# ZhiHuangHn/vtkCloudPoint

Hardware: AMD Instinct MI355X
Metric: Mpoints/s DBSCAN+label @10M pts (higher is better)
Workload: dtype f64; 1 GPU; C4: 10000000-pt cloud (half uniform background, 200 Gaussian blobs), one monolithic DBImproved.dbscan, metric L1_2D, eps 0.1, minPts 10; mode=single, points_total=10000000, points_per_gpu=10000000, clusters=27380, resident_in_hbm=True

## Files before the change

vtkcloudpoint_amd/csrc/dbscan.hip:

```cpp
#include <string.h>

#include <cmath>
#include <cstdlib>
#include <cstring>
#include <limits>
#include <vector>

#include "bounds.hpp"
#include "dbscan_engine.hpp"
#include "grid_common.hpp"

using namespace vcpg;

namespace {

#ifndef VCP_UNR2
#define VCP_UNR2 4
#endif
#ifndef VCP_UNR3
#define VCP_UNR3 2
#endif
#ifndef VCP_UNRW
#define VCP_UNRW 4
#endif

}

struct SlabState {
// ... 91 lines not shown
  for (int r = 0; r < NR; r++) {
    const int y = cc[1] + (r % 3) - 1;
    const int z = GD == 3 ? cc[2] + (r / 3) - 1 : 0;
    const bool ok = y >= 0 && y < g.D[1] && (GD != 3 || (z >= 0 && z < g.D[2]));
    const uint32_t base = ok ? cell_id<GD>(g, 0, y, z) : 0u;
    rs[r] = re[r] = 0u;
    if (ok) ct_range(ct, base + x0, base + x1 + 1, rs[r], re[r]);
  }
}

constexpr unsigned XCHUNK = 8;
constexpr unsigned LCHUNK = 1;
__device__ __forceinline__ int64_t xcd_block(unsigned nblocks) {
  const unsigned b = blockIdx.x;
  const unsigned per = nblocks / (8u * XCHUNK);
  if (b >= per * 8u * XCHUNK) return b;
  const unsigned x = b & 7u, i = b >> 3;
  return (int64_t)((i / per) * 8u + x) * per + (i % per);
}

struct WorkList {
  uint32_t* list;
  const uint32_t* scan;
  uint32_t perblk;
  uint32_t nblk;
};

__device__ __forceinline__ uint32_t wl_fetch(const WorkList& w) {
  const uint32_t total = w.scan[w.nblk] - w.scan[0];
  const uint32_t x = blockIdx.x & 7u, i = blockIdx.x >> 3;
  const uint32_t c = (i / w.perblk) * 8u + x;
  const uint32_t lo = (uint32_t)(((uint64_t)total * c) / (8u * LCHUNK));
  const uint32_t hi = (uint32_t)(((uint64_t)total * (c + 1u)) / (8u * LCHUNK));
  const uint32_t t = lo + (i % w.perblk) * TPB + threadIdx.x;
  if (t >= hi) return NONE;
  return w.list[t];
}

__device__ __forceinline__ void wl_count(bool isE, bool isB, uint32_t blk, uint32_t* __restrict__ cntE,
                                         uint32_t* __restrict__ cntB) {
  __shared__ unsigned wc[2][TPB / 64];
  const unsigned long long mE = __ballot(isE), mB = __ballot(isB);
  if ((threadIdx.x & 63) == 0) {
    wc[0][threadIdx.x >> 6] = (unsigned)__popcll(mE);
    wc[1][threadIdx.x >> 6] = (unsigned)__popcll(mB);
  }
  __syncthreads();
  if (threadIdx.x == 0) {
    unsigned a = 0, b = 0;
    for (int k = 0; k < TPB / 64; k++) {
      a += wc[0][k];
      b += wc[1][k];
    }
    cntE[blk] = a;
    cntB[blk] = b;
  }
}

__global__ __launch_bounds__(TPB) void k_wl_fill(const uint8_t* __restrict__ flags, CellTab ct, const uint32_t* __restrict__ scanE,
// ... 470 lines not shown
  for_rows<GD>(cc, g, ct, [&](uint32_t s, uint32_t e) {
    if (s >= me) return true;
    if (e > me) e = me;
    for (uint32_t j0 = s; j0 < e; j0 += UNR) {
      float rr[UNR][3];
      bool cand[UNR];
#pragma unroll
      for (int u = 0; u < UNR; u++) {
        const uint32_t jj = min(j0 + u, e - 1);
        cand[u] = (j0 + u < e) && (flags[jj] & F_EXPAND);
        if (GROUPED) cand[u] = cand[u] && sgroup[jj] == myg;
        load_pt32<GD>(sorted32, jj, rr[u]);
      }
#pragma unroll
      for (int u = 0; u < UNR; u++)
        if (first == me && cand[u] && within_scr<GD, METRIC>(qf, rr[u], sc, xs, me, j0 + u, thr)) first = j0 + u;
      if (first != me) return false;
    }
    return true;
  });
  if (first != me) parent[me] = first;
}

__global__ __launch_bounds__(TPB) void k_union_init_list(const uint8_t* __restrict__ flags, uint32_t* __restrict__ parent,
                                                        NbrOut no, WorkList wlE) {
  const uint32_t p = wl_fetch(wlE);
  if (p == NONE) return;
  const int nrec = flags[p] >> 4;
  const uint32_t* li = nbr_list(no, p);
  for (int k = 0; k < nrec; k++) {
    const uint32_t j = li[k];
    if (j < p && (flags[j] & F_EXPAND)) {
      parent[p] = j;
      return;
    }
  }
}

template <int JOIN>
__global__ __launch_bounds__(TPB) void k_flatten0(uint32_t* __restrict__ parent, WorkList wlE,
                                                 const uint8_t* __restrict__ flags, NbrOut no) {
  const uint32_t p = wl_fetch(wlE);
  if (p == NONE) return;
  uint32_t r = (uint32_t)p, x = ld_parent_cached(parent, r);
  if (x == r || JOIN == 2) {
    if (!JOIN) return;
    uint32_t rp = JOIN == 2 ? uf_root(parent, p) : p;
    const int nrec = flags[p] >> 4;
    const uint32_t* li = nbr_list(no, p);
    uint32_t s0 = NONE, s1 = NONE, s2 = NONE;
    for (int k = 0; k < nrec; k++) {
      const uint32_t j = li[k];
      if (!(flags[j] & F_EXPAND)) continue;
      const uint32_t y = ld_parent_cached(parent, j);
      if (y == rp || y == s0 || y == s1 || y == s2) continue;
      const uint32_t ry = uf_root(parent, y);
      const uint32_t rm = uf_root(parent, rp);
      s2 = s1;
      s1 = s0;
      s0 = rp;
      rp = (ry != rm) ? uf_link(parent, rm, ry) : rm;
      if (y != rp) s1 = y;
    }
    return;
  }
  while (x != r) {
    r = x;
    x = ld_parent_cached(parent, r);
  }
  __hip_atomic_store(&parent[p], r, __ATOMIC_RELAXED, __HIP_MEMORY_SCOPE_WAVEFRONT);
}

constexpr uint32_t CHUNK_MIXED = 0xFFFFFFFEu;
constexpr int DENSE_PER_CELL = 16;
__global__ __launch_bounds__(TPB) void k_chunkroot(const uint32_t* __restrict__ parent, CellTab ct,
                                                  uint32_t* __restrict__ chunkroot) {
  const uint32_t nin = *ct.nin;
  const int64_t p = (int64_t)blockIdx.x * TPB + threadIdx.x;
  const uint32_t x = p < nin ? parent[p] : NONE;
  const unsigned long long have = __ballot(x != NONE);
  uint32_t out = NONE;
  if (have) {
    const uint32_t r = (uint32_t)__shfl((int)x, __ffsll((long long)have) - 1, 64);
    out = __ballot(x != NONE && x != r) ? CHUNK_MIXED : r;
  }
  if ((threadIdx.x & 63) == 0) chunkroot[p >> 6] = out;
}

#define VCP_JOIN(x)                                                \
  do {                                                             \
    const uint32_t rx__ = uf_root(parent, (x));                    \
    const uint32_t rm__ = uf_root(parent, rp);                     \
    rp = (rx__ != rm__) ? uf_link(parent, rm__, rx__) : rm__;      \
// ... 74 lines not shown
          if (x2 != rp) {
            const uint32_t rx = uf_root(parent, x2);
            const uint32_t rm = uf_root(parent, rp);
            rp = (rx != rm) ? uf_link(parent, rm, rx) : rm;
          }
          if (x != rp && j != rp) __hip_atomic_store(&parent[j], rp, __ATOMIC_RELAXED, __HIP_MEMORY_SCOPE_WAVEFRONT);
        } else if (q0 == NONE) {
          q0 = x;
        } else if (q1 == NONE) {
          q1 = x;
        } else {
          VCP_FLUSH();
          q0 = x;
        }
      }
    }
  }
  VCP_FLUSH();
  if (rp != me) __hip_atomic_store(&parent[me], rp, __ATOMIC_RELAXED, __HIP_MEMORY_SCOPE_AGENT);
}
#undef VCP_FLUSH
#undef VCP_JOIN

template <bool FILTER>
__global__ __launch_bounds__(TPB) void k_flatten(uint32_t* __restrict__ parent, const uint32_t* __restrict__ sord,
                                                uint32_t* __restrict__ minord, WorkList wlE) {
  const uint32_t p = wl_fetch(wlE);
  uint32_t r = NONE, v = NONE;
  if (p != NONE) {
    r = (uint32_t)p;
    uint32_t x = parent[r];
    while (x != r) {
      r = x;
      x = parent[r];
    }
    parent[p] = r;
    v = sord[p];
  }
  unsigned long long todo = __ballot(r != NONE);
  const int lane = threadIdx.x & 63;
  while (todo) {
    int leader = __ffsll((long long)todo) - 1;
    uint32_t lr = __shfl(r, leader, 64);
    bool mine = (r == lr);
    uint32_t m = mine ? v : NONE;
#pragma unroll
    for (int d = 32; d > 0; d >>= 1) m = min(m, (uint32_t)__shfl_xor((int)m, d, 64));
    if (lane == leader &&
        (!FILTER || m < __hip_atomic_load(&minord[lr], __ATOMIC_RELAXED, __HIP_MEMORY_SCOPE_AGENT)))
      atomicMin(&minord[lr], m);
    todo &= ~__ballot(mine);
  }
}

__device__ __forceinline__ uint32_t seed_rank(const uint32_t* __restrict__ bits, const uint32_t* __restrict__ pref,
                                              uint32_t m) {
  const uint32_t w = m >> 5;
  return pref[w] + (uint32_t)__popc(bits[w] & ((1u << (m & 31u)) - 1u));
}
__global__ __launch_bounds__(TPB) void k_seed_popc(const uint32_t* __restrict__ bits, uint32_t nw, uint32_t* __restrict__ cnt) {
  uint32_t w = blockIdx.x * TPB + threadIdx.x;
  if (w < nw) cnt[w] = (uint32_t)__popc(bits[w]);
}

__global__ __launch_bounds__(TPB) void k_seedflag(const uint32_t* __restrict__ parent, const uint32_t* __restrict__ minord,
                                                 uint32_t* __restrict__ seedflag, WorkList wlE) {
  const uint32_t p = wl_fetch(wlE);
  if (p == NONE) return;
  if (parent[p] == p) {
    const uint32_t m = minord[p];
    atomicOr(&seedflag[m >> 5], 1u << (m & 31u));
  }
}

__global__ __launch_bounds__(TPB) void k_rootk(const uint32_t* __restrict__ parent, const uint32_t* __restrict__ minord,
                                              const uint32_t* __restrict__ seedbits, const uint32_t* __restrict__ seedpref,
                                              uint32_t* __restrict__ rootk, uint32_t* __restrict__ clseed, WorkList wlE) {
  const uint32_t p = wl_fetch(wlE);
  if (p == NONE) return;
  if (parent[p] == p) {
    uint32_t k = seed_rank(seedbits, seedpref, minord[p]);
    rootk[p] = k;
    clseed[k] = minord[p];
  }
}

__device__ __forceinline__ void twice_add(unsigned twice, unsigned long long* __restrict__ counters) {
  __shared__ unsigned tw[TPB / 64];
  const unsigned long long m2 = __ballot(twice);
  if ((threadIdx.x & 63) == 0) tw[threadIdx.x >> 6] = (unsigned)__popcll(m2);
  __syncthreads();
  if (threadIdx.x == 0) {
    unsigned t = 0;
    for (int k = 0; k < TPB / 64; k++) t += tw[k];
    if (t) atomicAdd(&counters[CNT_TWICE + (blockIdx.x & (CNT_SPREAD - 1))], (unsigned long long)t);
  }
}

template <int GD, int METRIC, bool GROUPED>
__global__ __launch_bounds__(TPB) void k_border(ExactSrc xs, GridP g, double thr,
                                               CellTab ct,
                                               const int32_t* __restrict__ sgroup, const uint8_t* __restrict__ flags,
                                               const uint32_t* __restrict__ parent, const uint32_t* __restrict__ sord,
                                               const uint32_t* __restrict__ rootk, const uint32_t* __restrict__ clseed,
                                               uint32_t* __restrict__ labk, unsigned long long* __restrict__ counters,
                                               uint32_t* __restrict__ group_twice, WorkList wlB, uint32_t own_lo,
                                               uint32_t own_span, const float* __restrict__ sorted32, Screen sc) {
  const uint32_t p = wl_fetch(wlB);
  unsigned twice = 0;
  if (p != NONE) {
    const uint8_t fl = flags[p];
    uint32_t out = 0;
    {
// ... 15 lines not shown
            if (j >= e || x == NONE || (x >= mnk && x < mx)) continue;
            if (GROUPED && sgroup[j] != myg) continue;
            float rr[3];
            load_pt32<GD>(sorted32, j, rr);
            if (within_scr<GD, METRIC>(qf, rr, sc, xs, p, j, thr)) {
              mx = max(mx, x + 1u);
              mnk = min(mnk, x);
            }
          }
        }
        return true;
      });
      out = mx;
      if (mx != 0 && !(fl & F_CLASSED) && sord[p] - own_lo < own_span && sord[p] < clseed[mnk]) {
        twice = 1;
        if (GROUPED) atomicAdd(&group_twice[myg], 1u);
      }
    }
    labk[p] = (out << 2) | ((fl & F_CORE) ? 1u : 0u) | ((fl & F_CLASSED) ? 2u : 0u);
  }
  if (!GROUPED) twice_add(twice, counters);
}

template <bool GROUPED>
__global__ __launch_bounds__(TPB) void k_border_list(const int32_t* __restrict__ sgroup, const uint8_t* __restrict__ flags,
                                                    const uint32_t* __restrict__ sord, const uint32_t* __restrict__ rootk,
                                                    const uint32_t* __restrict__ clseed, uint32_t* __restrict__ labk,
                                                    unsigned long long* __restrict__ counters,
                                                    uint32_t* __restrict__ group_twice, NbrOut no, WorkList wlB) {
  const uint32_t p = wl_fetch(wlB);
  unsigned twice = 0;
  if (p != NONE) {
    const uint8_t fl = flags[p];
    const int nrec = fl >> 4;
    uint32_t mx = 0, mnk = NONE;
    const uint32_t* li = nbr_list(no, p);
    for (int k = 0; k < nrec; k++) {
      const uint32_t x = rootk[li[k]];
      if (x == NONE) continue;
      mx = max(mx, x + 1u);
      mnk = min(mnk, x);
    }
    if (mx != 0 && sord[p] < clseed[mnk]) twice = 1;
    labk[p] = (mx << 2) | ((fl & F_CORE) ? 1u : 0u) | ((fl & F_CLASSED) ? 2u : 0u);
  }
  if (GROUPED) {
    const int32_t g = twice ? sgroup[p] : -1;
    unsigned long long todo = __ballot(twice != 0);
    const int lane = threadIdx.x & 63;
    while (todo) {
      const int leader = __ffsll((long long)todo) - 1;
      const int32_t gl = __shfl(g, leader, 64);
      const unsigned long long same = __ballot(twice && g == gl);
      if (lane == leader) atomicAdd(&group_twice[gl], (uint32_t)__popcll(same));
      todo &= ~same;
    }
  } else {
    twice_add(twice, counters);
  }
}

__global__ __launch_bounds__(TPB) void k_labk_rest(const uint8_t* __restrict__ flags, const uint32_t* __restrict__ parent,
                                                  uint32_t* rootk, uint32_t* __restrict__ labk,
                                                  CellTab ct) {
  const uint32_t nin = *ct.nin;
  int64_t p = (int64_t)blockIdx.x * TPB + threadIdx.x;
  if (p >= nin) return;
  const uint8_t fl = flags[p];
  uint32_t k = NONE;
  if (fl & F_EXPAND) {
    const uint32_t r = parent[p];
    k = rootk[r];
    if (r != (uint32_t)p) rootk[p] = k;
  } else {
    rootk[p] = NONE;
  }
  if (fl & F_BCAND) return;
  const uint32_t out = (fl & F_EXPAND) ? k + 1u : 0u;
  labk[p] = (out << 2) | ((fl & F_CORE) ? 1u : 0u) | ((fl & F_CLASSED) ? 2u : 0u);
}

// ... 223 lines not shown
  if (metric == VCP_L1_2D) {
    err = 2.0 * alpha * (1.0 + u) + 2.0 * u * (1.0 + u) * thr;
  } else {
    err = 2.0 * alpha * std::sqrt((double)gd * thr) * (1.0 + u) + (double)gd * alpha * alpha + 6.0 * u * (1.0 + u) * thr;
    lo_ok = std::sqrt(thr) > 4.0 * alpha * std::sqrt((double)gd);
  }
  err = err * 1.0625 + 1e-14 * thr + 1e-300;
  const double lo = thr - err, hi = thr + err;
  if (std::isfinite(hi)) {
    float h = (float)hi;
    if ((double)h < hi) h = std::nextafterf(h, INFINITY);
    sc.hi = h;
  }
  if (lo_ok && lo >= 0.0 && std::isfinite(lo)) {
    float l = (float)lo;
    if ((double)l > lo) l = std::nextafterf(l, -INFINITY);
    sc.lo = l;
  } else if (lo_ok && std::isinf(thr) && thr > 0) {
    sc.lo = 3.4028234663852886e38f;
  }
  return sc;
}

unsigned list_perblk(int64_t n) {
  const int64_t band = (n + 8 * LCHUNK - 1) / (8 * LCHUNK) + 1;
  return vcp_blocks(band, TPB);
}

struct Switches {
  int64_t cells_per_point;
  bool screen_off, lists_off, core_global;
  int core_cap, join_all;
};
const Switches& switches() {
  static const Switches sw = [] {
    Switches s;
    const char* e = getenv("VCP_CELL_BUDGET");
    const long v = e ? atol(e) : 32;
    s.cells_per_point = (int64_t)(v < 1 ? 1 : v > 4096 ? 4096 : v);
    s.screen_off = getenv("VCP_NO_SCREEN") != nullptr;
    s.lists_off = getenv("VCP_NO_LISTS") != nullptr;
    s.core_global = getenv("VCP_CORE_GLOBAL") != nullptr;
    s.core_cap = getenv("VCP_CORE_CAP") ? atoi(getenv("VCP_CORE_CAP")) : -1;
    s.join_all = getenv("VCP_JOIN_ALL") ? atoi(getenv("VCP_JOIN_ALL")) : -1;
    return s;
  }();
  return sw;
}

struct EnginePinned {
  double bounds[8];
  uint32_t unclassed;
  uint32_t n_comp;
  unsigned long long counters[CNT_WORDS];
};
static_assert(sizeof(EnginePinned) <= 1024, "the engine's region of vcp_ctx::pinned");
EnginePinned* engine_pinned(vcp_ctx* ctx) { return reinterpret_cast<EnginePinned*>(ctx->pinned); }

struct Call {
  const double* d_coords;
  int64_t n;
  int stride, metric;
  double eps;
  int min_pts;
  int32_t cf_in;
  const uint8_t* d_in_classed;
  int32_t* d_labels;
  uint8_t *d_is_core, *d_is_classed;
  int32_t* cf_out;
  int64_t* dist_evals;
// ... 29 lines not shown
}
BoundsSrc bounds_src(const Call& c) { return BoundsSrc{c.d_coords, c.n, c.gd, c.stride, c.d_group, c.glo, c.ghi}; }

struct MiscView {
  double* d_part;
  double* d_bounds;
  unsigned long long* counters;
  uint32_t* d_total;
};
struct Workspace : MiscView {
  uint4* ctwords;
  uint32_t* ctdense;
  uint32_t* ctcount;
  CellTab ct;
  uint32_t *cellof, *pos, *sord, *parent, *minord, *rootk, *clseed, *labk;
  float* sorted32;
  uint8_t* flags;
  int32_t* sgroup;
  uint32_t nw;
  uint32_t* seedflag;
  uint32_t* seedpref;
  uint32_t *blkE, *blkB;
  WorkList wlE, wlB;
  unsigned nbl;
};

int ws_reserve_misc(vcp_ctx* ctx, int64_t n) {
  return vcp_ensure(ctx, ctx->b_misc, (size_t)(vcp_bounds_parts(n) * 8 + 96) * sizeof(double));
}
MiscView misc_carve(vcp_ctx* ctx, int64_t n) {
  MiscView m;
  m.d_part = ctx->b_misc.as<double>();
  m.d_bounds = m.d_part + (size_t)vcp_bounds_parts(n) * 8;
  m.counters = reinterpret_cast<unsigned long long*>(m.d_bounds + 8);
  m.d_total = reinterpret_cast<uint32_t*>(m.counters + CNT_SEED_TOTAL);
  return m;
}
static_assert((8 + CNT_WORDS) <= 96, "b_misc: bounds and counters behind the partials");

int ws_reserve(vcp_ctx* ctx, int64_t n, unsigned nb, int gd, bool grouped, uint32_t ncells) {
  const size_t ctw = vcp_ct_words(ncells), ctd = vcp_ct_dense_cap(n, ncells);
  VCP_TRY(vcp_ensure(ctx, ctx->b_ctw, ctw * 16 + 64));
  VCP_TRY(vcp_ensure(ctx, ctx->b_ctd, ctd * 128));
  VCP_TRY(vcp_ensure(ctx, ctx->b_cellof, (size_t)n * 4));
  VCP_TRY(vcp_ensure(ctx, ctx->b_pos, (size_t)n * 4));
  VCP_TRY(vcp_ensure(ctx, ctx->b_sorted32, (size_t)n * (gd == 2 ? 2 : 4) * 4));
  VCP_TRY(vcp_ensure(ctx, ctx->b_sidx, (size_t)n * 4));
// ... 17 lines not shown
  w.ctcount = reinterpret_cast<uint32_t*>(ctx->b_ctw.as<char>() + vcp_ct_words(ncells) * 16);
  w.ct = CellTab{w.ctwords, w.ctdense, w.ctcount + 1};
  w.cellof = ctx->b_cellof.as<uint32_t>();
  w.pos = ctx->b_pos.as<uint32_t>();
  w.sorted32 = ctx->b_sorted32.as<float>();
  w.sord = ctx->b_sidx.as<uint32_t>();
  w.flags = ctx->b_flags.as<uint8_t>();
  w.parent = ctx->b_parent.as<uint32_t>();
  w.minord = ctx->b_minord.as<uint32_t>();
  w.nw = (uint32_t)(n / 32 + 2);
  w.seedflag = ctx->b_seedflag.as<uint32_t>();
  w.seedpref = w.seedflag + ((w.nw + 3) & ~3u);
  w.rootk = ctx->b_rootcl.as<uint32_t>();
  w.clseed = ctx->b_clseed.as<uint32_t>();
  w.labk = ctx->b_labk.as<uint32_t>();
  w.sgroup = grouped ? ctx->b_sgroup.as<int32_t>() : nullptr;
  w.blkE = ctx->b_wl.as<uint32_t>();
  w.blkB = w.blkE + (nb + 2);
  w.wlE.list = w.blkB + (nb + 2);
  w.wlB.list = w.wlE.list + n;
  w.wlE.scan = w.blkE;
  w.wlB.scan = w.blkB;
  w.wlE.nblk = w.wlB.nblk = nb;
  w.wlE.perblk = w.wlB.perblk = list_perblk(n);
  w.nbl = 8u * LCHUNK * w.wlE.perblk;
  return w;
}

struct Totals {
  uint32_t K;
  unsigned long long unclassed;
  unsigned long long twice;
  unsigned long long slot0;
  unsigned long long group_evals;
};
int read_totals(vcp_ctx* ctx, const MiscView& ws, Totals& t) {
  unsigned long long* hc = engine_pinned(ctx)->counters;
  VCP_HIP(ctx, hipMemcpyAsync(hc, ws.counters, CNT_WORDS * sizeof(unsigned long long), hipMemcpyDeviceToHost, ctx->stream));
  VCP_TRY(vcp_phase_finish(ctx));
  VCP_HIP(ctx, hipStreamSynchronize(ctx->stream));
  t.K = *reinterpret_cast<uint32_t*>(hc + CNT_SEED_TOTAL);
  t.slot0 = hc[CNT_LONELY];
  t.group_evals = hc[CNT_GROUP_EVALS];
  t.unclassed = t.twice = 0;
  for (int k = 0; k < CNT_SPREAD; k++) {
    t.unclassed += hc[CNT_UNCLASSED + k];
    t.twice += hc[CNT_TWICE + k];
  }
// ... 178 lines not shown
  }
  const size_t lds_nb = (size_t)no.NB * TPB * 4;
  bool tiled = false;
  if constexpr (GD == 2) {
    if (!GROUPED || !sw.core_global) {
      VCP_LAUNCH(ctx, (k_core_lds<GD, METRIC, GROUPED>), dim3(nb), dim3(TPB), 0, st, c.xs, c.g, c.thr, c.min_pts, ws.ct,
                      ws.sgroup, ws.flags, ws.parent, ws.minord, ws.blkE, ws.blkB, no, ws.sorted32, c.sc, c.flags_set);
      tiled = true;
    }
  }
  if (!tiled)
    VCP_LAUNCH(ctx, (k_core<GD, METRIC, GROUPED>), dim3(nb), dim3(TPB), 2 * lds_nb, st, c.xs, c.g, c.thr, c.min_pts, ws.ct,
                    ws.sgroup, ws.flags, ws.parent, ws.minord, ws.blkE, ws.blkB, no, ws.sorted32, c.sc, c.flags_set);
  VCP_TRY(vcp_exclusive_scan_u32(ctx, ws.blkE, ws.blkE, 2 * ((int64_t)nb + 2), nullptr));
  VCP_LAUNCH(ctx, k_wl_fill, dim3(nb), dim3(TPB), 0, st, ws.flags, ws.ct, ws.blkE, ws.blkB, ws.wlE.list, ws.wlB.list,
                  ws.seedflag, ws.nw, ws.counters, c.d_group_twice, (uint32_t)(GROUPED ? c.G : 0));
  return VCP_OK;
}

template <int GD, int METRIC, bool GROUPED>
int stage_union(vcp_ctx* ctx, const Call& c, const Workspace& ws, const Switches& sw) {
  hipStream_t st = ctx->stream;
  const int64_t n = c.n;
  const unsigned nb = c.nb, nbl = ws.nbl;
  const GridP& g = c.g;
  const NbrOut& no = c.no;
  vcp_phase(ctx, "union");
  const bool pre = GD == 2 || no.NB > 0;
  if (no.NB > 0) {
    VCP_LAUNCH(ctx, k_union_init_list, dim3(nbl), dim3(TPB), 0, st, ws.flags, ws.parent, no, ws.wlE);
    const bool all = sw.join_all >= 0 ? sw.join_all != 0 : (uint64_t)n >= (uint64_t)g.ncells;
    if (all) VCP_LAUNCH(ctx, k_flatten0<2>, dim3(nbl), dim3(TPB), 0, st, ws.parent, ws.wlE, ws.flags, no);
    else VCP_LAUNCH(ctx, k_flatten0<1>, dim3(nbl), dim3(TPB), 0, st, ws.parent, ws.wlE, ws.flags, no);
    VCP_LAUNCH(ctx, k_flatten0<0>, dim3(nbl), dim3(TPB), 0, st, ws.parent, ws.wlE, ws.flags, no);
  } else if (GD == 2) {
    VCP_LAUNCH(ctx, (k_union_init<GD, METRIC, GROUPED>), dim3(nbl), dim3(TPB), 0, st, c.xs, g, c.thr, ws.ct, ws.sgroup,
                    ws.flags, ws.parent, ws.wlE, ws.sorted32, c.sc);
    VCP_LAUNCH(ctx, k_flatten0<0>, dim3(nbl), dim3(TPB), 0, st, ws.parent, ws.wlE, ws.flags, no);
  }
  const bool dense = pre && (uint64_t)n > (uint64_t)DENSE_PER_CELL * g.ncells;
  if (dense) {
    VCP_TRY(vcp_ensure(ctx, ctx->b_aux0, ((size_t)nb * (TPB / 64) + 2) * 4));
    uint32_t* chunkroot = ctx->b_aux0.as<uint32_t>();
    VCP_LAUNCH(ctx, k_chunkroot, dim3(nb), dim3(TPB), 0, st, ws.parent, ws.ct, chunkroot);
    VCP_LAUNCH(ctx, (k_union<GD, METRIC, GROUPED, true, true>), dim3(nbl), dim3(TPB), 0, st, c.xs, g, c.thr, ws.ct,
                    ws.sgroup, ws.parent, ws.wlE, ws.sorted32, c.sc, chunkroot);
  } else if (pre)
    VCP_LAUNCH(ctx, (k_union<GD, METRIC, GROUPED, true>), dim3(nbl), dim3(TPB), 0, st, c.xs, g, c.thr, ws.ct, ws.sgroup,
                    ws.parent, ws.wlE, ws.sorted32, c.sc);
  else
    VCP_LAUNCH(ctx, (k_union<GD, METRIC, GROUPED, false>), dim3(nbl), dim3(TPB), 0, st, c.xs, g, c.thr, ws.ct, ws.sgroup,
                    ws.parent, ws.wlE, ws.sorted32, c.sc);
  return VCP_OK;
}

int stage_slab_handoff(vcp_ctx* ctx, const Call& c, const Workspace& ws) {
  hipStream_t st = ctx->stream;
  const unsigned nb = c.nb;
  vcp_phase(ctx, "slab_components");
  VCP_LAUNCH(ctx, k_slab_count, dim3(nb), dim3(TPB), 0, st, ws.parent, ws.flags, ws.ct, ws.blkE);
  VCP_TRY(vcp_exclusive_scan_u32(ctx, ws.blkE, ws.blkE, (int64_t)nb + 1, nullptr));
// ... 1 lines not shown
  VCP_LAUNCH(ctx, k_slab_out, dim3(nb), dim3(TPB), 0, st, c.n, ws.pos, ws.flags, ws.parent, ws.minord, c.ext->d_slab_rep,
                  c.d_is_core);
  uint32_t* hn = &engine_pinned(ctx)->n_comp;
  VCP_HIP(ctx, hipMemcpyAsync(hn, ws.blkE + nb, 4, hipMemcpyDeviceToHost, st));
  VCP_TRY(vcp_phase_finish(ctx));
  VCP_HIP(ctx, hipStreamSynchronize(st));
  if (!ctx->slab) ctx->slab = new SlabState();
  SlabState& ss = *ctx->slab;
  ss.valid = true;
  ss.gd = c.gd;
  ss.metric = c.metric;
  ss.n = c.n;
  ss.n_comp = hn[0];
  ss.g = c.g;
  ss.thr = c.thr;
  ss.sc = c.sc;
  ss.xs = c.xs;
  ss.nb = nb;
  if (c.cf_out) *c.cf_out = (int32_t)hn[0];
  return VCP_OK;
}

template <bool GROUPED>
int stage_flatten_number(vcp_ctx* ctx, const Call& c, const Workspace& ws) {
  hipStream_t st = ctx->stream;
  const unsigned nbl = ws.nbl;
  vcp_phase(ctx, "flatten_number");
  if ((uint64_t)c.n >= (uint64_t)c.g.ncells)
    VCP_LAUNCH(ctx, k_flatten<true>, dim3(nbl), dim3(TPB), 0, st, ws.parent, ws.sord, ws.minord, ws.wlE);
  else
    VCP_LAUNCH(ctx, k_flatten<false>, dim3(nbl), dim3(TPB), 0, st, ws.parent, ws.sord, ws.minord, ws.wlE);
  if (!GROUPED && c.slab) return stage_slab_handoff(ctx, c, ws);
  VCP_LAUNCH(ctx, k_seedflag, dim3(nbl), dim3(TPB), 0, st, ws.parent, ws.minord, ws.seedflag, ws.wlE);
  VCP_LAUNCH(ctx, k_seed_popc, dim3(vcp_blocks(ws.nw, TPB)), dim3(TPB), 0, st, ws.seedflag, ws.nw, ws.seedpref);
  VCP_TRY(vcp_exclusive_scan_u32(ctx, ws.seedpref, ws.seedpref, ws.nw, ws.d_total));
  VCP_LAUNCH(ctx, k_rootk, dim3(nbl), dim3(TPB), 0, st, ws.parent, ws.minord, ws.seedflag, ws.seedpref, ws.rootk, ws.clseed,
                  ws.wlE);
  return VCP_OK;
}

template <int GD, int METRIC, bool GROUPED>
int stage_border(vcp_ctx* ctx, const Call& c, const Workspace& ws) {
  hipStream_t st = ctx->stream;
  vcp_phase(ctx, "border");
  VCP_LAUNCH(ctx, k_labk_rest, dim3(c.nb), dim3(TPB), 0, st, ws.flags, ws.parent, ws.rootk, ws.labk, ws.ct);
  if (c.no.NB > 0)
    VCP_LAUNCH(ctx, k_border_list<GROUPED>, dim3(ws.nbl), dim3(TPB), 0, st, ws.sgroup, ws.flags, ws.sord, ws.rootk,
                    ws.clseed, ws.labk, ws.counters, c.d_group_twice, c.no, ws.wlB);
  else
    VCP_LAUNCH(ctx, (k_border<GD, METRIC, GROUPED>), dim3(ws.nbl), dim3(TPB), 0, st, c.xs, c.g, c.thr, ws.ct, ws.sgroup,
                    ws.flags, ws.parent, ws.sord, ws.rootk, ws.clseed, ws.labk, ws.counters, c.d_group_twice, ws.wlB, 0u,
                    NONE, ws.sorted32, c.sc);
  return VCP_OK;
}

template <int GD, bool GROUPED>
int stage_output(vcp_ctx* ctx, const Call& c, const Workspace& ws) {
  hipStream_t st = ctx->stream;
  const int64_t n = c.n;
  const unsigned nb = c.nb;
  const DbscanExt* ext = c.ext;
  if (c.part_out) {
    GridOutputArgs oa;
    oa.n = n;
    oa.sord = ws.sord;
    oa.labk = ws.labk;
    oa.have_in_classed = c.d_in_classed != nullptr;
    oa.cf_in = c.cf_in;
    oa.labels = c.d_labels;
    oa.is_core = c.d_is_core;
    oa.is_classed = c.d_is_classed;
    oa.counters = ws.counters;
    VCP_TRY(vcp_grid_output_partition(ctx, oa));
// ... 15 lines not shown
  }
  return VCP_OK;
}

template <int GD, int METRIC, bool GROUPED>
int run_dbscan(vcp_ctx* ctx, Call& c) {
  const Switches& sw = switches();
  VCP_TRY(stage_bounds(ctx, c));
  c.thr = (METRIC == VCP_L1_2D) ? c.eps : l2_threshold(c.eps);
  if (!GROUPED && c.all_finite && !c.slab && box_measure<GD, METRIC>(c.h) <= c.thr) return run_all_pairs(ctx, c);

  double Emax = 0.0;
  VCP_TRY(grid_geometry(ctx, c, sw, Emax));
  c.sc = screen_bounds(METRIC, GD, METRIC == VCP_L1_2D ? c.thr * c.g.scale : c.thr * c.g.scale * c.g.scale, Emax * c.g.scale);
  if (sw.screen_off) c.sc = Screen{-1.0f, INFINITY};

  VCP_TRY(ws_reserve(ctx, c.n, c.nb, GD, GROUPED, c.g.ncells));
  const Workspace ws = ws_carve(ctx, c.n, c.nb, GROUPED, c.g.ncells);
  c.flags_set = c.d_in_classed != nullptr;
  c.part_out = !GROUPED && !c.d_ord && !c.slab && c.n <= ((int64_t)1 << 27);
  VCP_TRY(stage_grid_build(ctx, c, ws));
  VCP_TRY((stage_core<GD, METRIC, GROUPED>(ctx, c, ws, sw)));
  VCP_TRY((stage_union<GD, METRIC, GROUPED>(ctx, c, ws, sw)));
  VCP_TRY(stage_flatten_number<GROUPED>(ctx, c, ws));
  if (!GROUPED && c.slab) return VCP_OK;
  VCP_TRY((stage_border<GD, METRIC, GROUPED>(ctx, c, ws)));
  VCP_TRY((stage_output<GD, GROUPED>(ctx, c, ws)));

  Totals t;
  VCP_TRY(read_totals(ctx, ws, t));
  const unsigned long long unclassed = c.d_in_classed ? t.unclassed : (unsigned long long)c.n;
  if (c.cf_out) *c.cf_out = c.cf_in + (int32_t)t.K;
  if (c.dist_evals)
    *c.dist_evals = GROUPED ? (int64_t)t.group_evals : (int64_t)(unclassed + t.twice + t.K - t.slot0) * c.n;
  return VCP_OK;
}

template <int GD, int METRIC>
int run_slab_finish(vcp_ctx* ctx, const SlabState& ss, const uint32_t* d_map_rep, const uint32_t* d_map_k,
                    const int32_t* d_tab_gid, uint32_t own_lo, uint32_t own_span, int32_t* d_labels,
                    uint8_t* d_is_classed, int64_t* twice) {
  hipStream_t st = ctx->stream;
  const int64_t n = ss.n;
  const unsigned nb = ss.nb;
  const Workspace ws = ws_carve(ctx, n, nb, false, ss.g.ncells);
  vcp_phase(ctx, "slab_roots");
  VCP_HIP(ctx, hipMemsetAsync(ws.counters, 0, CNT_WORDS * sizeof(unsigned long long), st));
  VCP_LAUNCH(ctx, k_slab_rootk, dim3(nb), dim3(TPB), 0, st, ws.parent, ws.flags, ws.minord, ws.ct, d_map_rep, d_map_k,
                  (uint32_t)ss.n_comp, ws.rootk, ws.counters + CNT_MISSING);
  vcp_phase(ctx, "border");
  VCP_LAUNCH(ctx, k_labk_rest, dim3(nb), dim3(TPB), 0, st, ws.flags, ws.parent, ws.rootk, ws.labk, ws.ct);
  VCP_LAUNCH(ctx, (k_border<GD, METRIC, false>), dim3(ws.nbl), dim3(TPB), 0, st, ss.xs, ss.g, ss.thr, ws.ct, nullptr,
                  ws.flags, ws.parent, ws.sord, ws.rootk, ws.clseed, ws.labk, ws.counters, nullptr, ws.wlB, own_lo,
                  own_span, ws.sorted32, ss.sc);
  vcp_phase(ctx, "output");
  VCP_LAUNCH(ctx, k_slab_output, dim3(nb), dim3(TPB), 0, st, n, ws.pos, ws.labk, d_tab_gid, d_labels, d_is_classed);
  Totals t;
  VCP_TRY(read_totals(ctx, ws, t));
  if (t.slot0 != 0)
    return vcp_fail(ctx, VCP_ERR_ARG, "%llu local components are missing from the map", t.slot0);
  if (twice) *twice = (int64_t)t.twice;
  return VCP_OK;
}

int run_degenerate(vcp_ctx* ctx, const Call& c) {
  hipStream_t st = ctx->stream;
  const int64_t n = c.n;
  vcp_phase(ctx, "degenerate");
  VCP_TRY(vcp_ensure(ctx, ctx->b_seedflag, (size_t)(n + 2) * 4));
  VCP_TRY(vcp_ensure(ctx, ctx->b_misc, 64));
  uint32_t* f = ctx->b_seedflag.as<uint32_t>();
  uint32_t* d_total = ctx->b_misc.as<uint32_t>();
  VCP_TRY(unclassed_ranks(ctx, c, f, d_total));
  const int all_core = 0 >= c.min_pts;
  VCP_LAUNCH(ctx, k_degenerate, dim3(c.nb), dim3(TPB), 0, st, c.d_in_classed, f, n, c.cf_in, all_core,
// ... 207 lines not shown
```

Before: 7034 Mpoints/s.

## Process multiple worklist entries per thread in union, flatten, seed and border kernels

Worklist kernels (union init, flatten0, flatten, seedflag, rootk, border_list) are templated on E, the number of worklist entries each thread handles, with their loads interleaved to raise memory-level parallelism. Grid sizes shrink to match, and E defaults to 4, capped at 2 for some kernels, with an environment switch to choose it. The aim is to hide the latency of dependent gather loads. The cost is more registers, lower occupancy and lanes that diverge on irregular loops.

```diff
diff --git a/vtkcloudpoint_amd/csrc/dbscan.hip b/vtkcloudpoint_amd/csrc/dbscan.hip
--- a/vtkcloudpoint_amd/csrc/dbscan.hip
+++ b/vtkcloudpoint_amd/csrc/dbscan.hip
@@ -4,6 +4,7 @@
 #include <cstdlib>
 #include <cstring>
 #include <limits>
+#include <type_traits>
 #include <vector>
 
 #include "bounds.hpp"
@@ -141,19 +142,27 @@
 struct WorkList {
   uint32_t* list;
   const uint32_t* scan;
-  uint32_t perblk;
+  uint32_t perblk[3];
   uint32_t nblk;
 };
-
-__device__ __forceinline__ uint32_t wl_fetch(const WorkList& w) {
+constexpr int wl_slot(int E) { return E == 4 ? 2 : E == 2 ? 1 : 0; }
+
+template <int E>
+__device__ __forceinline__ void wl_fetch(const WorkList& w, uint32_t (&p)[E]) {
   const uint32_t total = w.scan[w.nblk] - w.scan[0];
+  const uint32_t perblk = w.perblk[wl_slot(E)];
   const uint32_t x = blockIdx.x & 7u, i = blockIdx.x >> 3;
-  const uint32_t c = (i / w.perblk) * 8u + x;
+  const uint32_t c = (i / perblk) * 8u + x;
   const uint32_t lo = (uint32_t)(((uint64_t)total * c) / (8u * LCHUNK));
   const uint32_t hi = (uint32_t)(((uint64_t)total * (c + 1u)) / (8u * LCHUNK));
-  const uint32_t t = lo + (i % w.perblk) * TPB + threadIdx.x;
-  if (t >= hi) return NONE;
-  return w.list[t];
+  const uint32_t t = lo + (i % perblk) * (TPB * E) + threadIdx.x;
+#pragma unroll
+  for (int e = 0; e < E; e++) p[e] = t + e * TPB < hi ? w.list[t + e * TPB] : NONE;
+}
+__device__ __forceinline__ uint32_t wl_fetch(const WorkList& w) {
+  uint32_t p[1];
+  wl_fetch<1>(w, p);
+  return p[0];
 }
 
 __device__ __forceinline__ void wl_count(bool isE, bool isB, uint32_t blk, uint32_t* __restrict__ cntE,
@@ -670,53 +679,127 @@
   if (first != me) parent[me] = first;
 }
 
+
+template <int E>
+__device__ __forceinline__ void wl_lists(const uint8_t* __restrict__ flags, const NbrOut& no, const uint32_t (&p)[E],
+                                         const bool (&want)[E], uint8_t (&fl)[E], const uint32_t* (&li)[E]) {
+  uint16_t of[E];
+#pragma unroll
+  for (int e = 0; e < E; e++) {
+    fl[e] = want[e] ? flags[p[e]] : (uint8_t)0;
+    of[e] = want[e] ? no.off[p[e]] : (uint16_t)0;
+  }
+#pragma unroll
+  for (int e = 0; e < E; e++)
+    li[e] = want[e] ? no.nbr + (size_t)(p[e] / TPB) * (size_t)(no.NB * TPB) + of[e] : nullptr;
+}
+
+template <int E>
 __global__ __launch_bounds__(TPB) void k_union_init_list(const uint8_t* __restrict__ flags, uint32_t* __restrict__ parent,
                                                         NbrOut no, WorkList wlE) {
-  const uint32_t p = wl_fetch(wlE);
-  if (p == NONE) return;
-  const int nrec = flags[p] >> 4;
-  const uint32_t* li = nbr_list(no, p);
-  for (int k = 0; k < nrec; k++) {
-    const uint32_t j = li[k];
-    if (j < p && (flags[j] & F_EXPAND)) {
-      parent[p] = j;
-      return;
-    }
-  }
-}
-
-template <int JOIN>
+  uint32_t p[E];
+  wl_fetch<E>(wlE, p);
+  if (p[0] == NONE) return;
+  bool want[E];
+  uint8_t fl[E];
+  const uint32_t* li[E];
+  int nrec[E];
+#pragma unroll
+  for (int e = 0; e < E; e++) want[e] = p[e] != NONE;
+  wl_lists<E>(flags, no, p, want, fl, li);
+#pragma unroll
+  for (int e = 0; e < E; e++) nrec[e] = fl[e] >> 4;
+  for (int k = 0;; k++) {
+    bool on[E], any = false;
+    uint32_t j[E];
+    uint8_t fj[E];
+#pragma unroll
+    for (int e = 0; e < E; e++) any |= on[e] = k < nrec[e];
+    if (!any) break;
+#pragma unroll
+    for (int e = 0; e < E; e++) j[e] = on[e] ? li[e][k] : NONE;
+#pragma unroll
+    for (int e = 0; e < E; e++) fj[e] = (on[e] && j[e] < p[e]) ? flags[j[e]] : (uint8_t)0;
+#pragma unroll
+    for (int e = 0; e < E; e++)
+      if (fj[e] & F_EXPAND) {
+        parent[p[e]] = j[e];
+        nrec[e] = 0;
+      }
+  }
+}
+
+
+__device__ __forceinline__ void join_edge(uint32_t* parent, const uint8_t* __restrict__ flags, uint32_t j, uint32_t& rp,
+                                          uint32_t& s0, uint32_t& s1, uint32_t& s2) {
+  if (!(flags[j] & F_EXPAND)) return;
+  const uint32_t y = ld_parent_cached(parent, j);
+  if (y == rp || y == s0 || y == s1 || y == s2) return;
+  const uint32_t ry = uf_root(parent, y);
+  const uint32_t rm = uf_root(parent, rp);
+  s2 = s1;
+  s1 = s0;
+  s0 = rp;
+  rp = (ry != rm) ? uf_link(parent, rm, ry) : rm;
+  if (y != rp) s1 = y;
+}
+
+template <int JOIN, int E>
 __global__ __launch_bounds__(TPB) void k_flatten0(uint32_t* __restrict__ parent, WorkList wlE,
                                                  const uint8_t* __restrict__ flags, NbrOut no) {
-  const uint32_t p = wl_fetch(wlE);
-  if (p == NONE) return;
-  uint32_t r = (uint32_t)p, x = ld_parent_cached(parent, r);
-  if (x == r || JOIN == 2) {
-    if (!JOIN) return;
-    uint32_t rp = JOIN == 2 ? uf_root(parent, p) : p;
-    const int nrec = flags[p] >> 4;
-    const uint32_t* li = nbr_list(no, p);
-    uint32_t s0 = NONE, s1 = NONE, s2 = NONE;
-    for (int k = 0; k < nrec; k++) {
-      const uint32_t j = li[k];
-      if (!(flags[j] & F_EXPAND)) continue;
-      const uint32_t y = ld_parent_cached(parent, j);
-      if (y == rp || y == s0 || y == s1 || y == s2) continue;
-      const uint32_t ry = uf_root(parent, y);
-      const uint32_t rm = uf_root(parent, rp);
-      s2 = s1;
-      s1 = s0;
-      s0 = rp;
-      rp = (ry != rm) ? uf_link(parent, rm, ry) : rm;
-      if (y != rp) s1 = y;
-    }
-    return;
-  }
-  while (x != r) {
-    r = x;
-    x = ld_parent_cached(parent, r);
-  }
-  __hip_atomic_store(&parent[p], r, __ATOMIC_RELAXED, __HIP_MEMORY_SCOPE_WAVEFRONT);
+  uint32_t p[E];
+  wl_fetch<E>(wlE, p);
+  if (p[0] == NONE) return;
+  uint32_t r[E], x[E];
+  bool joins[E], chase[E], go[E], any = false;
+#pragma unroll
+  for (int e = 0; e < E; e++) {
+    r[e] = p[e];
+    x[e] = p[e] != NONE ? ld_parent_cached(parent, p[e]) : NONE;
+  }
+#pragma unroll
+  for (int e = 0; e < E; e++) {
+    joins[e] = JOIN && p[e] != NONE && (x[e] == r[e] || JOIN == 2);
+    chase[e] = go[e] = JOIN != 2 && x[e] != r[e];
+    any |= go[e];
+  }
+  while (any) {
+#pragma unroll
+    for (int e = 0; e < E; e++)
+      if (go[e]) {
+        r[e] = x[e];
+        x[e] = ld_parent_cached(parent, r[e]);
+      }
+    any = false;
+#pragma unroll
+    for (int e = 0; e < E; e++) any |= go[e] = go[e] && x[e] != r[e];
+  }
+#pragma unroll
+  for (int e = 0; e < E; e++)
+    if (chase[e]) __hip_atomic_store(&parent[p[e]], r[e], __ATOMIC_RELAXED, __HIP_MEMORY_SCOPE_WAVEFRONT);
+  if (!JOIN) return;
+  uint8_t fl[E];
+  const uint32_t* li[E];
+  uint32_t rp[E], s0[E], s1[E], s2[E];
+  wl_lists<E>(flags, no, p, joins, fl, li);
+#pragma unroll
+  for (int e = 0; e < E; e++) {
+    rp[e] = (JOIN == 2 && joins[e]) ? uf_root(parent, p[e]) : p[e];
+    s0[e] = s1[e] = s2[e] = NONE;
+  }
+  for (int k = 0;; k++) {
+    bool on[E];
+    uint32_t j[E];
+    any = false;
+#pragma unroll
+    for (int e = 0; e < E; e++) any |= on[e] = k < (fl[e] >> 4);
+    if (!any) break;
+#pragma unroll
+    for (int e = 0; e < E; e++) j[e] = on[e] ? li[e][k] : NONE;
+#pragma unroll
+    for (int e = 0; e < E; e++)
+      if (on[e]) join_edge(parent, flags, j[e], rp[e], s0[e], s1[e], s2[e]);
+  }
 }
 
 constexpr uint32_t CHUNK_MIXED = 0xFFFFFFFEu;
@@ -837,34 +920,51 @@
 #undef VCP_FLUSH
 #undef VCP_JOIN
 
-template <bool FILTER>
+template <bool FILTER, int E>
 __global__ __launch_bounds__(TPB) void k_flatten(uint32_t* __restrict__ parent, const uint32_t* __restrict__ sord,
                                                 uint32_t* __restrict__ minord, WorkList wlE) {
-  const uint32_t p = wl_fetch(wlE);
-  uint32_t r = NONE, v = NONE;
-  if (p != NONE) {
-    r = (uint32_t)p;
-    uint32_t x = parent[r];
-    while (x != r) {
-      r = x;
-      x = parent[r];
-    }
-    parent[p] = r;
-    v = sord[p];
-  }
-  unsigned long long todo = __ballot(r != NONE);
+  uint32_t p[E];
+  wl_fetch<E>(wlE, p);
+  uint32_t r[E], x[E], v[E];
+  bool go[E], any = false;
+#pragma unroll
+  for (int e = 0; e < E; e++) {
+    r[e] = p[e];
+    x[e] = p[e] != NONE ? parent[p[e]] : NONE;
+    v[e] = p[e] != NONE ? sord[p[e]] : NONE;
+  }
+#pragma unroll
+  for (int e = 0; e < E; e++) any |= go[e] = x[e] != r[e];
+  while (any) {
+#pragma unroll
+    for (int e = 0; e < E; e++)
+      if (go[e]) {
+        r[e] = x[e];
+        x[e] = parent[r[e]];
+      }
+    any = false;
+#pragma unroll
+    for (int e = 0; e < E; e++) any |= go[e] = go[e] && x[e] != r[e];
+  }
+#pragma unroll
+  for (int e = 0; e < E; e++)
+    if (p[e] != NONE) parent[p[e]] = r[e];
   const int lane = threadIdx.x & 63;
-  while (todo) {
-    int leader = __ffsll((long long)todo) - 1;
-    uint32_t lr = __shfl(r, leader, 64);
-    bool mine = (r == lr);
-    uint32_t m = mine ? v : NONE;
-#pragma unroll
-    for (int d = 32; d > 0; d >>= 1) m = min(m, (uint32_t)__shfl_xor((int)m, d, 64));
-    if (lane == leader &&
-        (!FILTER || m < __hip_atomic_load(&minord[lr], __ATOMIC_RELAXED, __HIP_MEMORY_SCOPE_AGENT)))
-      atomicMin(&minord[lr], m);
-    todo &= ~__ballot(mine);
+#pragma unroll
+  for (int e = 0; e < E; e++) {
+    unsigned long long todo = __ballot(r[e] != NONE);
+    while (todo) {
+      int leader = __ffsll((long long)todo) - 1;
+      uint32_t lr = __shfl(r[e], leader, 64);
+      bool mine = (r[e] == lr);
+      uint32_t m = mine ? v[e] : NONE;
+#pragma unroll
+      for (int d = 32; d > 0; d >>= 1) m = min(m, (uint32_t)__shfl_xor((int)m, d, 64));
+      if (lane == leader &&
+          (!FILTER || m < __hip_atomic_load(&minord[lr], __ATOMIC_RELAXED, __HIP_MEMORY_SCOPE_AGENT)))
+        atomicMin(&minord[lr], m);
+      todo &= ~__ballot(mine);
+    }
   }
 }
 
@@ -878,32 +978,61 @@
   if (w < nw) cnt[w] = (uint32_t)__popc(bits[w]);
 }
 
+template <int E>
+__device__ __forceinline__ void wl_roots(const uint32_t* __restrict__ parent, const uint32_t* __restrict__ minord,
+                                         const uint32_t (&p)[E], bool (&root)[E], uint32_t (&m)[E]) {
+  uint32_t x[E];
+#pragma unroll
+  for (int e = 0; e < E; e++) x[e] = p[e] != NONE ? parent[p[e]] : 0u;
+#pragma unroll
+  for (int e = 0; e < E; e++) root[e] = x[e] == p[e];
+#pragma unroll
+  for (int e = 0; e < E; e++) m[e] = root[e] ? minord[p[e]] : NONE;
+}
+
+template <int E>
 __global__ __launch_bounds__(TPB) void k_seedflag(const uint32_t* __restrict__ parent, const uint32_t* __restrict__ minord,
                                                  uint32_t* __restrict__ seedflag, WorkList wlE) {
-  const uint32_t p = wl_fetch(wlE);
-  if (p == NONE) return;
-  if (parent[p] == p) {
-    const uint32_t m = minord[p];
-    atomicOr(&seedflag[m >> 5], 1u << (m & 31u));
-  }
-}
-
+  uint32_t p[E], m[E];
+  bool root[E];
+  wl_fetch<E>(wlE, p);
+  if (p[0] == NONE) return;
+  wl_roots<E>(parent, minord, p, root, m);
+#pragma unroll
+  for (int e = 0; e < E; e++)
+    if (root[e]) atomicOr(&seedflag[m[e] >> 5], 1u << (m[e] & 31u));
+}
+
+template <int E>
 __global__ __launch_bounds__(TPB) void k_rootk(const uint32_t* __restrict__ parent, const uint32_t* __restrict__ minord,
                                               const uint32_t* __restrict__ seedbits, const uint32_t* __restrict__ seedpref,
                                               uint32_t* __restrict__ rootk, uint32_t* __restrict__ clseed, WorkList wlE) {
-  const uint32_t p = wl_fetch(wlE);
-  if (p == NONE) return;
-  if (parent[p] == p) {
-    uint32_t k = seed_rank(seedbits, seedpref, minord[p]);
-    rootk[p] = k;
-    clseed[k] = minord[p];
-  }
-}
-
+  uint32_t p[E], m[E], pf[E], bt[E];
+  bool root[E];
+  wl_fetch<E>(wlE, p);
+  if (p[0] == NONE) return;
+  wl_roots<E>(parent, minord, p, root, m);
+#pragma unroll
+  for (int e = 0; e < E; e++) {
+    pf[e] = root[e] ? seedpref[m[e] >> 5] : 0u;
+    bt[e] = root[e] ? seedbits[m[e] >> 5] : 0u;
+  }
+#pragma unroll
+  for (int e = 0; e < E; e++)
+    if (root[e]) {
+      const uint32_t k = pf[e] + (uint32_t)__popc(bt[e] & ((1u << (m[e] & 31u)) - 1u));
+      rootk[p[e]] = k;
+      clseed[k] = m[e];
+    }
+}
+
+template <int BITS = 1>
 __device__ __forceinline__ void twice_add(unsigned twice, unsigned long long* __restrict__ counters) {
   __shared__ unsigned tw[TPB / 64];
-  const unsigned long long m2 = __ballot(twice);
-  if ((threadIdx.x & 63) == 0) tw[threadIdx.x >> 6] = (unsigned)__popcll(m2);
+  unsigned wsum = 0;
+#pragma unroll
+  for (int b = 0; b < BITS; b++) wsum += (unsigned)__popcll(__ballot((twice >> b) & 1u)) << b;
+  if ((threadIdx.x & 63) == 0) tw[threadIdx.x >> 6] = wsum;
   __syncthreads();
   if (threadIdx.x == 0) {
     unsigned t = 0;
@@ -965,41 +1094,74 @@
   if (!GROUPED) twice_add(twice, counters);
 }
 
-template <bool GROUPED>
+template <bool GROUPED, int E>
 __global__ __launch_bounds__(TPB) void k_border_list(const int32_t* __restrict__ sgroup, const uint8_t* __restrict__ flags,
                                                     const uint32_t* __restrict__ sord, const uint32_t* __restrict__ rootk,
                                                     const uint32_t* __restrict__ clseed, uint32_t* __restrict__ labk,
                                                     unsigned long long* __restrict__ counters,
                                                     uint32_t* __restrict__ group_twice, NbrOut no, WorkList wlB) {
-  const uint32_t p = wl_fetch(wlB);
-  unsigned twice = 0;
-  if (p != NONE) {
-    const uint8_t fl = flags[p];
-    const int nrec = fl >> 4;
-    uint32_t mx = 0, mnk = NONE;
-    const uint32_t* li = nbr_list(no, p);
-    for (int k = 0; k < nrec; k++) {
-      const uint32_t x = rootk[li[k]];
-      if (x == NONE) continue;
-      mx = max(mx, x + 1u);
-      mnk = min(mnk, x);
-    }
-    if (mx != 0 && sord[p] < clseed[mnk]) twice = 1;
-    labk[p] = (mx << 2) | ((fl & F_CORE) ? 1u : 0u) | ((fl & F_CLASSED) ? 2u : 0u);
+  uint32_t p[E];
+  wl_fetch<E>(wlB, p);
+  bool want[E], twice[E];
+  uint8_t fl[E];
+  const uint32_t* li[E];
+  uint32_t mx[E], mnk[E];
+#pragma unroll
+  for (int e = 0; e < E; e++) {
+    want[e] = p[e] != NONE;
+    mx[e] = 0;
+    mnk[e] = NONE;
+  }
+  wl_lists<E>(flags, no, p, want, fl, li);
+  for (int k = 0;; k++) {
+    bool on[E], any = false;
+    uint32_t j[E], x[E];
+#pragma unroll
+    for (int e = 0; e < E; e++) any |= on[e] = k < (fl[e] >> 4);
+    if (!any) break;
+#pragma unroll
+    for (int e = 0; e < E; e++) j[e] = on[e] ? li[e][k] : NONE;
+#pragma unroll
+    for (int e = 0; e < E; e++) x[e] = on[e] ? rootk[j[e]] : NONE;
+#pragma unroll
+    for (int e = 0; e < E; e++)
+      if (x[e] != NONE) {
+        mx[e] = max(mx[e], x[e] + 1u);
+        mnk[e] = min(mnk[e], x[e]);
+      }
+  }
+  {
+    uint32_t so[E], cs[E];
+#pragma unroll
+    for (int e = 0; e < E; e++) {
+      so[e] = mx[e] != 0 ? sord[p[e]] : 0u;
+      cs[e] = mx[e] != 0 ? clseed[mnk[e]] : 0u;
+    }
+#pragma unroll
+    for (int e = 0; e < E; e++) {
+      twice[e] = so[e] < cs[e];
+      if (want[e]) labk[p[e]] = (mx[e] << 2) | ((fl[e] & F_CORE) ? 1u : 0u) | ((fl[e] & F_CLASSED) ? 2u : 0u);
+    }
   }
   if (GROUPED) {
-    const int32_t g = twice ? sgroup[p] : -1;
-    unsigned long long todo = __ballot(twice != 0);
     const int lane = threadIdx.x & 63;
-    while (todo) {
-      const int leader = __ffsll((long long)todo) - 1;
-      const int32_t gl = __shfl(g, leader, 64);
-      const unsigned long long same = __ballot(twice && g == gl);
-      if (lane == leader) atomicAdd(&group_twice[gl], (uint32_t)__popcll(same));
-      todo &= ~same;
+#pragma unroll
+    for (int e = 0; e < E; e++) {
+      const int32_t g = twice[e] ? sgroup[p[e]] : -1;
+      unsigned long long todo = __ballot(twice[e]);
+      while (todo) {
+        const int leader = __ffsll((long long)todo) - 1;
+        const int32_t gl = __shfl(g, leader, 64);
+        const unsigned long long same = __ballot(twice[e] && g == gl);
+        if (lane == leader) atomicAdd(&group_twice[gl], (uint32_t)__popcll(same));
+        todo &= ~same;
+      }
     }
   } else {
-    twice_add(twice, counters);
+    unsigned n2 = 0;
+#pragma unroll
+    for (int e = 0; e < E; e++) n2 += twice[e];
+    twice_add<E == 4 ? 3 : E>(n2, counters);
   }
 }
 
@@ -1269,15 +1431,16 @@
   return sc;
 }
 
-unsigned list_perblk(int64_t n) {
+unsigned list_perblk(int64_t n, int E) {
   const int64_t band = (n + 8 * LCHUNK - 1) / (8 * LCHUNK) + 1;
-  return vcp_blocks(band, TPB);
+  return vcp_blocks(band, (int64_t)TPB * E);
 }
 
 struct Switches {
   int64_t cells_per_point;
   bool screen_off, lists_off, core_global;
   int core_cap, join_all;
+  int wl_entries;
 };
 const Switches& switches() {
   static const Switches sw = [] {
@@ -1290,9 +1453,22 @@
     s.core_global = getenv("VCP_CORE_GLOBAL") != nullptr;
     s.core_cap = getenv("VCP_CORE_CAP") ? atoi(getenv("VCP_CORE_CAP")) : -1;
     s.join_all = getenv("VCP_JOIN_ALL") ? atoi(getenv("VCP_JOIN_ALL")) : -1;
+    const int wle = getenv("VCP_WL_ENTRIES") ? atoi(getenv("VCP_WL_ENTRIES")) : 4;
+    s.wl_entries = (wle == 1 || wle == 2) ? wle : 4;
     return s;
   }();
   return sw;
+}
+
+constexpr int WL_CAP = 2;
+constexpr int wl_capped(int E) { return E < WL_CAP ? E : WL_CAP; }
+template <class F>
+int wl_dispatch(int entries, F&& f) {
+  switch (entries) {
+    case 1: return f(std::integral_constant<int, 1>{});
+    case 2: return f(std::integral_constant<int, 2>{});
+    default: return f(std::integral_constant<int, 4>{});
+  }
 }
 
 struct EnginePinned {
@@ -1368,7 +1544,7 @@
   uint32_t* seedpref;
   uint32_t *blkE, *blkB;
   WorkList wlE, wlB;
-  unsigned nbl;
+  unsigned nbl[3];
 };
 
 int ws_reserve_misc(vcp_ctx* ctx, int64_t n) {
@@ -1432,8 +1608,11 @@
   w.wlE.scan = w.blkE;
   w.wlB.scan = w.blkB;
   w.wlE.nblk = w.wlB.nblk = nb;
-  w.wlE.perblk = w.wlB.perblk = list_perblk(n);
-  w.nbl = 8u * LCHUNK * w.wlE.perblk;
+  for (int E = 1; E <= 4; E *= 2) {
+    const int s = wl_slot(E);
+    w.wlE.perblk[s] = w.wlB.perblk[s] = list_perblk(n, E);
+    w.nbl[s] = 8u * LCHUNK * w.wlE.perblk[s];
+  }
   return w;
 }
 
@@ -1658,21 +1837,30 @@
 int stage_union(vcp_ctx* ctx, const Call& c, const Workspace& ws, const Switches& sw) {
   hipStream_t st = ctx->stream;
   const int64_t n = c.n;
-  const unsigned nb = c.nb, nbl = ws.nbl;
+  const unsigned nb = c.nb, nbl = ws.nbl[0];
   const GridP& g = c.g;
   const NbrOut& no = c.no;
   vcp_phase(ctx, "union");
   const bool pre = GD == 2 || no.NB > 0;
   if (no.NB > 0) {
-    VCP_LAUNCH(ctx, k_union_init_list, dim3(nbl), dim3(TPB), 0, st, ws.flags, ws.parent, no, ws.wlE);
     const bool all = sw.join_all >= 0 ? sw.join_all != 0 : (uint64_t)n >= (uint64_t)g.ncells;
-    if (all) VCP_LAUNCH(ctx, k_flatten0<2>, dim3(nbl), dim3(TPB), 0, st, ws.parent, ws.wlE, ws.flags, no);
-    else VCP_LAUNCH(ctx, k_flatten0<1>, dim3(nbl), dim3(TPB), 0, st, ws.parent, ws.wlE, ws.flags, no);
-    VCP_LAUNCH(ctx, k_flatten0<0>, dim3(nbl), dim3(TPB), 0, st, ws.parent, ws.wlE, ws.flags, no);
+    VCP_TRY(wl_dispatch(sw.wl_entries, [&](auto ec) {
+      constexpr int E = decltype(ec)::value, EC = wl_capped(E);
+      const dim3 gl(ws.nbl[wl_slot(E)]), glc(ws.nbl[wl_slot(EC)]);
+      VCP_LAUNCH(ctx, k_union_init_list<EC>, glc, dim3(TPB), 0, st, ws.flags, ws.parent, no, ws.wlE);
+      if (all) VCP_LAUNCH(ctx, (k_flatten0<2, EC>), glc, dim3(TPB), 0, st, ws.parent, ws.wlE, ws.flags, no);
+      else VCP_LAUNCH(ctx, (k_flatten0<1, EC>), glc, dim3(TPB), 0, st, ws.parent, ws.wlE, ws.flags, no);
+      VCP_LAUNCH(ctx, (k_flatten0<0, E>), gl, dim3(TPB), 0, st, ws.parent, ws.wlE, ws.flags, no);
+      return (int)VCP_OK;
+    }));
   } else if (GD == 2) {
     VCP_LAUNCH(ctx, (k_union_init<GD, METRIC, GROUPED>), dim3(nbl), dim3(TPB), 0, st, c.xs, g, c.thr, ws.ct, ws.sgroup,
                     ws.flags, ws.parent, ws.wlE, ws.sorted32, c.sc);
-    VCP_LAUNCH(ctx, k_flatten0<0>, dim3(nbl), dim3(TPB), 0, st, ws.parent, ws.wlE, ws.flags, no);
+    VCP_TRY(wl_dispatch(sw.wl_entries, [&](auto ec) {
+      constexpr int E = decltype(ec)::value;
+      VCP_LAUNCH(ctx, (k_flatten0<0, E>), dim3(ws.nbl[wl_slot(E)]), dim3(TPB), 0, st, ws.parent, ws.wlE, ws.flags, no);
+      return (int)VCP_OK;
+    }));
   }
   const bool dense = pre && (uint64_t)n > (uint64_t)DENSE_PER_CELL * g.ncells;
   if (dense) {
@@ -1720,33 +1908,46 @@
 }
 
 template <bool GROUPED>
-int stage_flatten_number(vcp_ctx* ctx, const Call& c, const Workspace& ws) {
+int stage_flatten_number(vcp_ctx* ctx, const Call& c, const Workspace& ws, const Switches& sw) {
   hipStream_t st = ctx->stream;
-  const unsigned nbl = ws.nbl;
   vcp_phase(ctx, "flatten_number");
-  if ((uint64_t)c.n >= (uint64_t)c.g.ncells)
-    VCP_LAUNCH(ctx, k_flatten<true>, dim3(nbl), dim3(TPB), 0, st, ws.parent, ws.sord, ws.minord, ws.wlE);
-  else
-    VCP_LAUNCH(ctx, k_flatten<false>, dim3(nbl), dim3(TPB), 0, st, ws.parent, ws.sord, ws.minord, ws.wlE);
+  VCP_TRY(wl_dispatch(sw.wl_entries, [&](auto ec) {
+    constexpr int E = wl_capped(decltype(ec)::value);
+    const dim3 gl(ws.nbl[wl_slot(E)]);
+    if ((uint64_t)c.n >= (uint64_t)c.g.ncells)
+      VCP_LAUNCH(ctx, (k_flatten<true, E>), gl, dim3(TPB), 0, st, ws.parent, ws.sord, ws.minord, ws.wlE);
+    else
+      VCP_LAUNCH(ctx, (k_flatten<false, E>), gl, dim3(TPB), 0, st, ws.parent, ws.sord, ws.minord, ws.wlE);
+    return (int)VCP_OK;
+  }));
   if (!GROUPED && c.slab) return stage_slab_handoff(ctx, c, ws);
-  VCP_LAUNCH(ctx, k_seedflag, dim3(nbl), dim3(TPB), 0, st, ws.parent, ws.minord, ws.seedflag, ws.wlE);
-  VCP_LAUNCH(ctx, k_seed_popc, dim3(vcp_blocks(ws.nw, TPB)), dim3(TPB), 0, st, ws.seedflag, ws.nw, ws.seedpref);
-  VCP_TRY(vcp_exclusive_scan_u32(ctx, ws.seedpref, ws.seedpref, ws.nw, ws.d_total));
-  VCP_LAUNCH(ctx, k_rootk, dim3(nbl), dim3(TPB), 0, st, ws.parent, ws.minord, ws.seedflag, ws.seedpref, ws.rootk, ws.clseed,
-                  ws.wlE);
+  VCP_TRY(wl_dispatch(sw.wl_entries, [&](auto ec) {
+    constexpr int E = decltype(ec)::value;
+    const dim3 gl(ws.nbl[wl_slot(E)]);
+    VCP_LAUNCH(ctx, k_seedflag<E>, gl, dim3(TPB), 0, st, ws.parent, ws.minord, ws.seedflag, ws.wlE);
+    VCP_LAUNCH(ctx, k_seed_popc, dim3(vcp_blocks(ws.nw, TPB)), dim3(TPB), 0, st, ws.seedflag, ws.nw, ws.seedpref);
+    VCP_TRY(vcp_exclusive_scan_u32(ctx, ws.seedpref, ws.seedpref, ws.nw, ws.d_total));
+    VCP_LAUNCH(ctx, k_rootk<E>, gl, dim3(TPB), 0, st, ws.parent, ws.minord, ws.seedflag, ws.seedpref, ws.rootk, ws.clseed,
+                    ws.wlE);
+    return (int)VCP_OK;
+  }));
   return VCP_OK;
 }
 
 template <int GD, int METRIC, bool GROUPED>
-int stage_border(vcp_ctx* ctx, const Call& c, const Workspace& ws) {
+int stage_border(vcp_ctx* ctx, const Call& c, const Workspace& ws, const Switches& sw) {
   hipStream_t st = ctx->stream;
   vcp_phase(ctx, "border");
   VCP_LAUNCH(ctx, k_labk_rest, dim3(c.nb), dim3(TPB), 0, st, ws.flags, ws.parent, ws.rootk, ws.labk, ws.ct);
   if (c.no.NB > 0)
-    VCP_LAUNCH(ctx, k_border_list<GROUPED>, dim3(ws.nbl), dim3(TPB), 0, st, ws.sgroup, ws.flags, ws.sord, ws.rootk,
-                    ws.clseed, ws.labk, ws.counters, c.d_group_twice, c.no, ws.wlB);
+    VCP_TRY(wl_dispatch(sw.wl_entries, [&](auto ec) {
+      constexpr int E = wl_capped(decltype(ec)::value);
+      VCP_LAUNCH(ctx, (k_border_list<GROUPED, E>), dim3(ws.nbl[wl_slot(E)]), dim3(TPB), 0, st, ws.sgroup, ws.flags, ws.sord,
+                      ws.rootk, ws.clseed, ws.labk, ws.counters, c.d_group_twice, c.no, ws.wlB);
+      return (int)VCP_OK;
+    }));
   else
-    VCP_LAUNCH(ctx, (k_border<GD, METRIC, GROUPED>), dim3(ws.nbl), dim3(TPB), 0, st, c.xs, c.g, c.thr, ws.ct, ws.sgroup,
+    VCP_LAUNCH(ctx, (k_border<GD, METRIC, GROUPED>), dim3(ws.nbl[0]), dim3(TPB), 0, st, c.xs, c.g, c.thr, ws.ct, ws.sgroup,
                     ws.flags, ws.parent, ws.sord, ws.rootk, ws.clseed, ws.labk, ws.counters, c.d_group_twice, ws.wlB, 0u,
                     NONE, ws.sorted32, c.sc);
   return VCP_OK;
@@ -1808,9 +2009,9 @@
   VCP_TRY(stage_grid_build(ctx, c, ws));
   VCP_TRY((stage_core<GD, METRIC, GROUPED>(ctx, c, ws, sw)));
   VCP_TRY((stage_union<GD, METRIC, GROUPED>(ctx, c, ws, sw)));
-  VCP_TRY(stage_flatten_number<GROUPED>(ctx, c, ws));
+  VCP_TRY(stage_flatten_number<GROUPED>(ctx, c, ws, sw));
   if (!GROUPED && c.slab) return VCP_OK;
-  VCP_TRY((stage_border<GD, METRIC, GROUPED>(ctx, c, ws)));
+  VCP_TRY((stage_border<GD, METRIC, GROUPED>(ctx, c, ws, sw)));
   VCP_TRY((stage_output<GD, GROUPED>(ctx, c, ws)));
 
   Totals t;
@@ -1836,7 +2037,7 @@
                   (uint32_t)ss.n_comp, ws.rootk, ws.counters + CNT_MISSING);
   vcp_phase(ctx, "border");
   VCP_LAUNCH(ctx, k_labk_rest, dim3(nb), dim3(TPB), 0, st, ws.flags, ws.parent, ws.rootk, ws.labk, ws.ct);
-  VCP_LAUNCH(ctx, (k_border<GD, METRIC, false>), dim3(ws.nbl), dim3(TPB), 0, st, ss.xs, ss.g, ss.thr, ws.ct, nullptr,
+  VCP_LAUNCH(ctx, (k_border<GD, METRIC, false>), dim3(ws.nbl[0]), dim3(TPB), 0, st, ss.xs, ss.g, ss.thr, ws.ct, nullptr,
                   ws.flags, ws.parent, ws.sord, ws.rootk, ws.clseed, ws.labk, ws.counters, nullptr, ws.wlB, own_lo,
                   own_span, ws.sorted32, ss.sc);
   vcp_phase(ctx, "output");
```

Result: faster. 7304 Mpoints/s (median of 6 runs) (+3.8%).
